# xuanvinh1997/llm-fp8

Hardware: AMD Instinct MI355X
Metric: train tokens/sec + FP8 GEMM % of MFMA peak, Llama-3.2-3B seq512 b16 (higher is better)
Workload: dtype fp8 (E4M3/E5M2 operands, fp32 accumulate, bf16 activations); 1 GPU; llama-3.2-3b (28 layers) full fine-tuning step, batch 16/GPU x seq 512, fp8_scenario=default (te_llama counterpart, lm_head FP8 under the outer recipe), random-init weights, synthetic tokens; route=fused, global_batch=16, seq_len=512, parallelism=single

## Files before the change

### include/mi_fp8.h

```cpp
#ifndef MI_FP8_H
#define MI_FP8_H

#include <stdint.h>

#ifdef __cplusplus
extern "C" {
#endif

#define MI_FMT_E4M3 0
#define MI_FMT_E5M2 1

#define MI_OK 0
#define MI_ERR_ARG (-1)
#define MI_ERR_SHAPE (-2)
#define MI_ERR_HIP (-3)

#define MI_OUT_BF16 0
#define MI_OUT_F32 1

#define MI_AMAX_ALGO_MAX 0
#define MI_AMAX_ALGO_MOST_RECENT 1

#define MI_ABI_VERSION 5
#define MI_ABI_REVISION 4
// ... 124 lines not shown
                        const float* grad_scale, float lr, float beta1, float beta2, float eps, float weight_decay,
                        int64_t step, void* stream);
int mi_adamw_cast_bf16_multi(const int64_t* table, int n_tensors, const int32_t* chunks, int n_chunks, int chunk_elems,
                             const float* grad_scale, float lr, float beta1, float beta2, float eps, float weight_decay,
                             int64_t step, void* stream);
int mi_adamw_mxcast_bf16_multi(const int64_t* table, int n_tensors, const int32_t* chunks, int n_chunks, int chunk_elems,
                               const float* grad_scale, float lr, float beta1, float beta2, float eps, float weight_decay,
                               int64_t step, void* stream);

int mi_adamw_f32_multi(const int64_t* table, int n_tensors, const int32_t* chunks, int n_chunks, int chunk_elems,
                       const float* grad_scale, float lr, float beta1, float beta2, float eps, float weight_decay,
                       int64_t step, int sink_kind, void* stream);

int mi_adamw_sr_bf16_multi(const int64_t* table, int n_tensors, const int32_t* chunks, int n_chunks, int chunk_elems,
                           const float* grad_scale, float lr, float beta1, float beta2, float eps, float weight_decay,
                           int64_t step, int sink_kind, uint64_t seed, void* stream);

int mi_embedding_grad_add(void* grad_bf16, const void* dy_bf16, const int64_t* sorted_ids, const int64_t* perm, int64_t tokens,
                          int64_t hidden, int64_t vocab, float alpha, int64_t padding_idx, void* stream);
int mi_adamw_bf16(void* p_bf16, const void* g_bf16, void* exp_avg_bf16, void* exp_avg_sq_bf16, int64_t n,
                  const float* grad_scale, float lr, float beta1, float beta2, float eps, float weight_decay,
                  int64_t step, void* stream);

int mi_attn_fwd(const void* q, const void* k, const void* v, void* o, float* lse, int B, int S, int H, int G, int D,
                int64_t q_ts, int64_t k_ts, int64_t v_ts, int64_t o_ts, float scale, int causal, void* stream);
typedef struct mi_gemm_plan {
  int algo, family, build, sched, mx, tile_cfg, tiles_m, tiles_n, grid_x, grid_y, block, one_tile_per_wg, sk_units, bias_use;
} mi_gemm_plan;
#ifdef MI_DIAG
int mi_attn_fwd_diag(const void* q, const void* k, const void* v, void* o, float* lse, unsigned long long* dbg, int B, int S,
                     int H, int G, int D, int64_t q_ts, int64_t k_ts, int64_t v_ts, int64_t o_ts, float scale, void* stream);
int mi_gemm_plan_diag(int entry, int64_t M, int64_t N, int64_t K, int64_t lda, int64_t ldb, int64_t ldd, int fmt_a, int fmt_b,
                      int out_dtype, int has_bias, int algo, mi_gemm_plan* out);
#endif
int mi_attn_bwd(const void* q, const void* k, const void* v, const void* o, const void* dout, const float* lse,
                float* delta, void* dq, void* dk, void* dv, int B, int S, int H, int G, int D, int64_t q_ts,
                int64_t k_ts, int64_t v_ts, int64_t o_ts, int64_t do_ts, int64_t dq_ts, int64_t dk_ts, int64_t dv_ts,
                float scale, int causal, void* stream);

#ifdef __cplusplus
}
#endif
#endif
```

### llm_fp8_amd/_lib.py

```python
from __future__ import annotations

import ctypes
import os

_HERE = os.path.dirname(os.path.abspath(__file__))
LIB_PATH = os.environ.get("LLM_FP8_AMD_LIB") or os.path.join(_HERE, "libmi_fp8.so")
LAB_LIB_PATH = os.path.join(os.path.dirname(_HERE), "tools", "bin", "libmi_fp8_lab.so")

MI_FMT_E4M3 = 0
MI_FMT_E5M2 = 1
ABI_VERSION = 5
ABI_REVISION = 4

_c_i64 = ctypes.c_int64
_c_int = ctypes.c_int
_p = ctypes.c_void_p

class GemmProblem(ctypes.Structure):
    _fields_ = [("A", ctypes.c_void_p), ("B", ctypes.c_void_p), ("D", ctypes.c_void_p), ("sa_inv", ctypes.c_void_p),
                ("sb_inv", ctypes.c_void_p), ("M", ctypes.c_int64), ("N", ctypes.c_int64), ("K", ctypes.c_int64),
                ("lda", ctypes.c_int64), ("ldb", ctypes.c_int64), ("ldd", ctypes.c_int64)]


class GemmMxProblem(ctypes.Structure):
# ... 48 lines not shown
    "mi_gemm_set_workspace": [_p, _c_i64],
    "mi_attn_fwd": [_p, _p, _p, _p, _p, _c_int, _c_int, _c_int, _c_int, _c_int, _c_i64, _c_i64, _c_i64, _c_i64, ctypes.c_float,
                    _c_int, _p],
    "mi_attn_bwd": [_p] * 10 + [_c_int] * 5 + [_c_i64] * 8 + [ctypes.c_float, _c_int, _p],
    "mi_mxfp8_norm_quantize": [_p, _p, _p, _p, _p, _p, _p, _c_i64, _c_i64, _c_int, _p],
    "mi_mxfp8_swiglu_quantize": [_p, _p, _p, _p, _p, _c_i64, _c_i64, _c_int, _p],
    "mi_mxfp8_dswiglu_quantize": [_p, _p, _p, _p, _p, _p, _p, _c_i64, _c_i64, _c_int, _p],
    "mi_gemm_mxfp8": [_p, _p, _p, _p, _p, _p, _c_i64, _c_i64, _c_i64, _c_int, _c_int, _c_int, _c_int, _p],
    "mi_swiglu_cast_bias": [_p, _p, _p, _p, _p, _p, _c_i64, _c_i64, _c_int, _p],
    "mi_dswiglu_cast_bias": [_p, _p, _p, _p, _p, _p, _p, _p, _c_i64, _c_i64, _c_int, _p],
    "mi_add_bias_rmsnorm_stats": [_p, _p, _p, _p, _p, _c_i64, _c_i64, ctypes.c_float, _p],
    "mi_gemm_fp8_clock": [_p, _p, _p, _p, _p, _c_i64, _c_i64, _c_i64, _c_i64, _c_i64, _c_i64, _c_int, _p, _p],
}
REVISION_SIGNATURES = {
    "mi_abi_revision": [],
    "mi_adamw_f32_multi": [_p, _c_int, _p, _c_int, _c_int, _p, ctypes.c_float, ctypes.c_float, ctypes.c_float, ctypes.c_float,
                           ctypes.c_float, _c_i64, _c_int, _p],
    "mi_amax_bf16": [_p, _p, _c_int, _c_i64, _c_i64, _p],
    "mi_amax_norm": [_p, _p, _p, _p, _c_int, _c_i64, _c_i64, _p],
    "mi_amax_swiglu": [_p, _p, _p, _c_int, _c_i64, _c_i64, _p],
    "mi_amax_dswiglu": [_p, _p, _p, _p, _c_int, _c_i64, _c_i64, _p],
    "mi_current_scale": [_p, _c_int, ctypes.c_float, ctypes.c_float, _c_int, _p, _p],
    "mi_blockfp8_quantize_ex": [_p, _p, _p, _p, _p, _p, _c_i64, _c_i64, _c_i64, _c_int, _c_int, ctypes.c_float, _p],
    "mi_blockfp8_norm_quantize": [_p, _p, _p, _p, _p, _p, _p, _c_i64, _c_i64, _c_int, _c_int, ctypes.c_float, _p],
    "mi_blockfp8_swiglu_quantize": [_p, _p, _p, _p, _p, _c_i64, _c_i64, _c_int, _c_int, ctypes.c_float, _p],
    "mi_blockfp8_dswiglu_quantize": [_p, _p, _p, _p, _p, _p, _p, _c_i64, _c_i64, _c_int, _c_int, ctypes.c_float, _p],
    "mi_adamw_sr_bf16_multi": [_p, _c_int, _p, _c_int, _c_int, _p, ctypes.c_float, ctypes.c_float, ctypes.c_float, ctypes.c_float,
                               ctypes.c_float, _c_i64, _c_int, ctypes.c_uint64, _p],
}
SIGNATURES.update(REVISION_SIGNATURES)
LAB_SIGNATURES = {
    "mi_attn_fwd_diag": [_p, _p, _p, _p, _p, _p, _c_int, _c_int, _c_int, _c_int, _c_int, _c_i64, _c_i64, _c_i64, _c_i64, ctypes.c_float, _p],
    "mi_gemm_plan_diag": [_c_int] + [_c_i64] * 6 + [_c_int] * 5 + [ctypes.POINTER(GemmPlan)],
}

_lib = None


def _bind(path: str, signatures) -> ctypes.CDLL:
    lib = ctypes.CDLL(path)
    for name, argtypes in signatures.items():
        if name in REVISION_SIGNATURES and not hasattr(lib, name):
            continue
        fn = getattr(lib, name)
        fn.argtypes = argtypes
        fn.restype = ctypes.c_char_p if name == "mi_last_error" else (_c_i64 if name == "mi_gemm_workspace_bytes" else _c_int)
    v = lib.mi_abi_version()
    if v != ABI_VERSION:
        raise ImportError(f"{os.path.basename(path)} ABI version {v} != expected {ABI_VERSION}; rebuild it")
    return lib


def load() -> ctypes.CDLL:
    global _lib
    if _lib is not None:
        return _lib
    if not os.path.exists(LIB_PATH):
        raise ImportError(
            f"{LIB_PATH} not found: the HIP extension is not built. Run "
            "`python -c 'import __graft_entry__ as g; g.build()'` or `make -C llm_fp8_amd/csrc`. "
            "llm_fp8_amd has no CPU/PyTorch fallback for the FP8 path.")
    _lib = _bind(LIB_PATH, SIGNATURES)
    return _lib


def use_lab_library() -> ctypes.CDLL:
# ... 31 lines not shown
```

### llm_fp8_amd/csrc/mi_api.hip

```cpp
#include "mi_common.h"
#include <string.h>

namespace mi {

static thread_local char g_err[512] = "";

void set_error(const char* fmt, ...) {
  va_list ap;
  va_start(ap, fmt);
  vsnprintf(g_err, sizeof(g_err), fmt, ap);
  va_end(ap);
}

int hip_fail(hipError_t e, const char* what) {
  set_error("%s: HIP error %d (%s)", what, (int)e, hipGetErrorString(e));
  return MI_ERR_HIP;
}

}

extern "C" int mi_abi_version(void) { return MI_ABI_VERSION; }
extern "C" int mi_abi_revision(void) { return MI_ABI_REVISION; }

extern "C" const char* mi_last_error(void) { return mi::g_err; }

extern "C" int mi_device_supported(void) {
  int dev = 0;
  hipError_t e = hipGetDevice(&dev);
  if (e != hipSuccess) return mi::hip_fail(e, "hipGetDevice");
  hipDeviceProp_t prop;
  e = hipGetDeviceProperties(&prop, dev);
  if (e != hipSuccess) return mi::hip_fail(e, "hipGetDeviceProperties");
  return strncmp(prop.gcnArchName, "gfx950", 6) == 0 ? 1 : 0;
}
```

### llm_fp8_amd/csrc/mi_common.h

```cpp
#pragma once
#include <hip/hip_runtime.h>
#include <float.h>
#include <stdint.h>
#include <stdio.h>
#include <stdarg.h>
#include "../../include/mi_fp8.h"

namespace mi {

void set_error(const char* fmt, ...);
int hip_fail(hipError_t e, const char* what);

#define MI_CHECK_AS(rc, cond, ...)         \
  do {                                     \
    if (!(cond)) {                         \
      mi::set_error(__VA_ARGS__);          \
      return rc;                           \
    }                                      \
  } while (0)
#define MI_CHECK_ARG(cond, ...) MI_CHECK_AS(MI_ERR_ARG, cond, __VA_ARGS__)
#define MI_CHECK_SHAPE(cond, ...) MI_CHECK_AS(MI_ERR_SHAPE, cond, __VA_ARGS__)

#define MI_CHECK_LAUNCH(what)                                   \
  do {                                                          \
// ... 25 lines not shown

template <int FMT>
__device__ __forceinline__ u32 cvt_pk_fp8(float a, float b) {
  const float mx = fp8_max_of<FMT>();
  a = __builtin_amdgcn_fmed3f(a, -mx, mx);
  b = __builtin_amdgcn_fmed3f(b, -mx, mx);
  if (FMT == MI_FMT_E4M3) return (u32)__builtin_amdgcn_cvt_pk_fp8_f32(a, b, 0, false) & 0xFFFFu;
  return (u32)__builtin_amdgcn_cvt_pk_bf8_f32(a, b, 0, false) & 0xFFFFu;
}

template <int FMT>
__device__ __forceinline__ u32 cvt4_fp8(float v0, float v1, float v2, float v3) {
  const float mx = fp8_max_of<FMT>();
  float c0 = __builtin_amdgcn_fmed3f(v0, -mx, mx), c1 = __builtin_amdgcn_fmed3f(v1, -mx, mx);
  float c2 = __builtin_amdgcn_fmed3f(v2, -mx, mx), c3 = __builtin_amdgcn_fmed3f(v3, -mx, mx);
  int r = 0;
  if (FMT == MI_FMT_E4M3) {
    r = __builtin_amdgcn_cvt_pk_fp8_f32(c0, c1, r, false);
    r = __builtin_amdgcn_cvt_pk_fp8_f32(c2, c3, r, true);
  } else {
    r = __builtin_amdgcn_cvt_pk_bf8_f32(c0, c1, r, false);
    r = __builtin_amdgcn_cvt_pk_bf8_f32(c2, c3, r, true);
  }
  u32 u = (u32)r;
  if (__builtin_expect((v0 != v0) | (v1 != v1) | (v2 != v2) | (v3 != v3), 0)) {
    if (v0 != v0) u = (u & 0xFFFFFF00u) | 0x0000007Fu;
    if (v1 != v1) u = (u & 0xFFFF00FFu) | 0x00007F00u;
    if (v2 != v2) u = (u & 0xFF00FFFFu) | 0x007F0000u;
    if (v3 != v3) u = (u & 0x00FFFFFFu) | 0x7F000000u;
  }
  return u;
}

typedef unsigned short u16x2 __attribute__((ext_vector_type(2)));
__device__ __forceinline__ u32 nan_screen(u32 acc, u32 w) {
  u16x2 a = __builtin_bit_cast(u16x2, acc), b = __builtin_bit_cast(u16x2, w & 0x7FFF7FFFu);
  return __builtin_bit_cast(u32, __builtin_elementwise_max(a, b));
}
__device__ __forceinline__ bool nan_seen(u32 acc) { return max(acc & 0xFFFFu, acc >> 16) > 0x7F80u; }

__device__ __forceinline__ u32 bperm(u32 hi, u32 lo, u32 sel) { return __builtin_amdgcn_perm(hi, lo, sel); }

__device__ __forceinline__ void transpose4x4(u32 r0, u32 r1, u32 r2, u32 r3, u32& c0, u32& c1, u32& c2,
                                             u32& c3) {
  u32 t01l = bperm(r1, r0, 0x05010400u);
  u32 t01h = bperm(r1, r0, 0x07030602u);
  u32 t23l = bperm(r3, r2, 0x05010400u);
  u32 t23h = bperm(r3, r2, 0x07030602u);
  c0 = bperm(t23l, t01l, 0x05040100u);
  c1 = bperm(t23l, t01l, 0x07060302u);
  c2 = bperm(t23h, t01h, 0x05040100u);
  c3 = bperm(t23h, t01h, 0x07060302u);
}

__device__ __forceinline__ u32 e8m0_roundup(float val) {
  u32 u = __float_as_uint(val);
  u32 e = (u >> 23) & 0xFFu, man = u & 0x7FFFFFu;
  if (man > 0 && e != 0xFEu && !(e == 0 && man <= 0x400000u)) ++e;
  if (val != val) e = 0xFFu;
  else if (isinf(val)) e = 0xFEu;
  else if (val == 0.0f) e = 0u;
  return e;
}
__device__ __forceinline__ float e8m0_inv(u32 e) {
  if (e == 0xFFu) return __uint_as_float(0x7FC00000u);
  if (e == 0xFEu) return __uint_as_float(0x00400000u);
  return __uint_as_float((254u - e) << 23);
}

__device__ __forceinline__ float scale_from_amax(float amax, float fp8_max, float eps, bool pow2) {
  const float a = amax < eps ? eps : amax;
  float scale = 1.0f;
  if (!(a == 0.0f) && !isinf(a)) {
    scale = fp8_max / a;
    if (isinf(scale)) scale = FLT_MAX;
    if (scale != scale) scale = 1.0f;
  }
  if (pow2) scale = __uint_as_float(__float_as_uint(scale) & 0xFF800000u);
  return scale;
}

__device__ __forceinline__ float wave_max(float v) {
#pragma unroll
  for (int o = 32; o >= 1; o >>= 1) v = fmaxf(v, __shfl_xor(v, o));
  return v;
}

__device__ __forceinline__ float sigmoidf_(float g) { return 1.0f / (1.0f + __expf(-g)); }

__device__ __forceinline__ void norm_value2(u32 w, float rs, float g0, float g1, float& v0, float& v1) {
  v0 = (__uint_as_float(w << 16) * rs) * g0;
  v1 = (__uint_as_float(w & 0xFFFF0000u) * rs) * g1;
}

template <int MODE>
__device__ __forceinline__ void swiglu_value2(u32 wg, u32 wu, u32 wd, bool has_bias, const float* bg, const float* bu, float* v0,
                                              float* v1) {
  float g2[2] = {__uint_as_float(wg << 16), __uint_as_float(wg & 0xFFFF0000u)};
  float u2[2] = {__uint_as_float(wu << 16), __uint_as_float(wu & 0xFFFF0000u)};
  const float d2[2] = {__uint_as_float(wd << 16), __uint_as_float(wd & 0xFFFF0000u)};
  if (has_bias) {
    g2[0] += bg[0];
    g2[1] += bg[1];
    u2[0] += bu[0];
    u2[1] += bu[1];
  }
#pragma unroll
  for (int e = 0; e < 2; ++e) {
    const float sg = sigmoidf_(g2[e]);
    if (MODE == 0) {
      v0[e] = g2[e] * sg * u2[e];
    } else {
      v0[e] = d2[e] * u2[e] * (sg * (1.0f + g2[e] * (1.0f - sg)));
      v1[e] = d2[e] * (g2[e] * sg);
    }
  }
}

}
#ifndef MI_NT_Y
#define MI_NT_Y 0
#endif
#ifndef MI_NT_YT
#define MI_NT_YT 0
#endif
#if defined(__HIPCC__)
namespace mi {
template <bool NT>
__device__ __forceinline__ void st8(uint8_t* p, unsigned int a, unsigned int b) {
  typedef unsigned int v2u_st8 __attribute__((ext_vector_type(2)));
  const v2u_st8 w = {a, b};
  if (NT) __builtin_nontemporal_store(w, reinterpret_cast<v2u_st8*>(p));
  else *reinterpret_cast<v2u_st8*>(p) = w;
}

template <bool NT>
__device__ __forceinline__ void store_rows8(uint8_t* dst, int64_t ld, const u32 (&lo)[8], const u32 (&hi)[8]) {
#pragma unroll
  for (int i = 0; i < 8; ++i) st8<NT>(dst + i * ld, lo[i], hi[i]);
}
template <bool NT>
__device__ __forceinline__ void store_cols8(uint8_t* dst, int64_t ld, const u32 (&lo)[8], const u32 (&hi)[8]) {
// ... 106 lines not shown
```

### llm_fp8_amd/csrc/mi_fused.hip

```cpp
#include "mi_common.h"

namespace mi {

template <int DIR>
__global__ __launch_bounds__(256) void rope_qkv_kernel(uint16_t* __restrict__ fused, uint16_t* __restrict__ q,
                                                       uint16_t* __restrict__ k, uint16_t* __restrict__ v,
                                                       const float* __restrict__ cosT, const float* __restrict__ sinT,
                                                       int rows, int seq, int nq, int nk, int D) {
  const int half = D >> 1;
  const int vph = half >> 3;
  const int W = (nq + 2 * nk) * D;
  const int rot_items = (nq + nk) * vph;
  const int cpy_items = (nk * D) >> 3;
  const int per_row = rot_items + cpy_items;
  const int64_t items = (int64_t)rows * per_row;
  const float sgn = DIR == 0 ? 1.0f : -1.0f;
  for (int64_t it = (int64_t)blockIdx.x * blockDim.x + threadIdx.x; it < items; it += (int64_t)gridDim.x * blockDim.x) {
    const int64_t r = it / per_row;
    const int w = (int)(it - r * per_row);
    uint16_t* frow = fused + r * W;
    if (w < rot_items) {
      const int hd = w / vph, vv = w - hd * vph;
      uint16_t* sep = hd < nq ? q + (r * nq + hd) * D : k + (r * nk + (hd - nq)) * D;
      uint16_t* f1 = frow + hd * D + vv * 8;
// ... 8 lines not shown
      *reinterpret_cast<v4f*>(c) = *reinterpret_cast<const v4f*>(cp);
      *reinterpret_cast<v4f*>(c + 4) = *reinterpret_cast<const v4f*>(cp + 4);
      *reinterpret_cast<v4f*>(sn) = *reinterpret_cast<const v4f*>(sp);
      *reinterpret_cast<v4f*>(sn + 4) = *reinterpret_cast<const v4f*>(sp + 4);
      v4i o1, o2;
#pragma unroll
      for (int j = 0; j < 4; ++j) {
        const u32 wa = (u32)a[j], wb = (u32)b[j];
        const float x1l = __uint_as_float(wa << 16), x1h = __uint_as_float(wa & 0xFFFF0000u);
        const float x2l = __uint_as_float(wb << 16), x2h = __uint_as_float(wb & 0xFFFF0000u);
        const float cl = c[2 * j], ch = c[2 * j + 1], sl = sgn * sn[2 * j], sh = sgn * sn[2 * j + 1];
        o1[j] = (int)pack_bf16x2(x1l * cl - x2l * sl, x1h * ch - x2h * sh);
        o2[j] = (int)pack_bf16x2(x2l * cl + x1l * sl, x2h * ch + x1h * sh);
      }
      *reinterpret_cast<v4i*>(out1) = o1;
      *reinterpret_cast<v4i*>(out1 + half) = o2;
    } else {
      const int cv = w - rot_items;
      uint16_t* fp = frow + (nq + nk) * D + cv * 8;
      uint16_t* sp2 = v + r * (int64_t)(nk * D) + cv * 8;
      if (DIR == 0) *reinterpret_cast<v4i*>(sp2) = *reinterpret_cast<const v4i*>(fp);
      else *reinterpret_cast<v4i*>(fp) = *reinterpret_cast<const v4i*>(sp2);
    }
  }
}

template <int FMT, bool WRITE_Y, bool WRITE_T>
__global__ __launch_bounds__(256) void rope_bwd_cast_kernel(const uint16_t* __restrict__ dq, const uint16_t* __restrict__ dk,
                                                            const uint16_t* __restrict__ dv, const float* __restrict__ cosT,
                                                            const float* __restrict__ sinT, uint8_t* __restrict__ y,
                                                            uint8_t* __restrict__ yT, const float* __restrict__ scale_p,
                                                            float* amax_out, int rows, int seq, int nq, int nk) {
  constexpr int D = 128, half = 64;
  __shared__ float s_amax[4];
  const int tid = threadIdx.x, lane = tid & 63, wave = tid >> 6;
  const int W = (nq + 2 * nk) * D;
  const int units = (nq + nk) + 2 * nk;
  const int64_t u_all = (int64_t)blockIdx.x * 4 + wave;
  const int rb = (int)(u_all / units), u = (int)(u_all % units);
  const int r0 = rb * 64 + (lane >> 3) * 8, lc = (lane & 7) * 8;
  const float scale = *scale_p;
  float amax = 0.0f;
  auto emit = [&](const float (&f)[8][8], int c0) {
    u32 lo[8], hi[8];
#pragma unroll
    for (int i = 0; i < 8; ++i) {
#pragma unroll
      for (int j = 0; j < 8; ++j) amax = fmaxf(amax, (f[i][j] != f[i][j]) ? 0.0f : fabsf(f[i][j]));
      lo[i] = cvt4_fp8<FMT>(f[i][0] * scale, f[i][1] * scale, f[i][2] * scale, f[i][3] * scale);
      hi[i] = cvt4_fp8<FMT>(f[i][4] * scale, f[i][5] * scale, f[i][6] * scale, f[i][7] * scale);
    }
    if (WRITE_Y) {
      uint8_t* dst = y + (int64_t)r0 * W + c0;
#pragma unroll
      for (int i = 0; i < 8; ++i) mi::st8<MI_NT_Y>(dst + (int64_t)i * W, lo[i], hi[i]);
    }
    if (WRITE_T) {
      u32 a[4], b[4], c[4], d[4];
      transpose4x4(lo[0], lo[1], lo[2], lo[3], a[0], a[1], a[2], a[3]);
      transpose4x4(lo[4], lo[5], lo[6], lo[7], b[0], b[1], b[2], b[3]);
      transpose4x4(hi[0], hi[1], hi[2], hi[3], c[0], c[1], c[2], c[3]);
      transpose4x4(hi[4], hi[5], hi[6], hi[7], d[0], d[1], d[2], d[3]);
      uint8_t* dst = yT + (int64_t)c0 * rows + r0;
#pragma unroll
      for (int j = 0; j < 4; ++j) {
        mi::st8<MI_NT_YT>(dst + (int64_t)j * rows, a[j], b[j]);
        mi::st8<MI_NT_YT>(dst + (int64_t)(j + 4) * rows, c[j], d[j]);
      }
    }
  };
  auto bf16_round = [](float v) { return __uint_as_float(float_to_bf16_bits(v) << 16); };
  if (r0 < rows) {
    if (u < nq + nk) {
      const int hd = u;
      const uint16_t* src = hd < nq ? dq + ((int64_t)r0 * nq + hd) * D : dk + ((int64_t)r0 * nk + (hd - nq)) * D;
      const int64_t rstride = (int64_t)(hd < nq ? nq : nk) * D;
      float f1[8][8], f2[8][8];
#pragma unroll
      for (int i = 0; i < 8; ++i) {
        const v4i a = *reinterpret_cast<const v4i*>(src + i * rstride + lc);
        const v4i b = *reinterpret_cast<const v4i*>(src + i * rstride + half + lc);
        const int pos = (r0 + i) % seq;
        float c[8], sn[8];
        *reinterpret_cast<v4f*>(c) = *reinterpret_cast<const v4f*>(cosT + (int64_t)pos * half + lc);
        *reinterpret_cast<v4f*>(c + 4) = *reinterpret_cast<const v4f*>(cosT + (int64_t)pos * half + lc + 4);
        *reinterpret_cast<v4f*>(sn) = *reinterpret_cast<const v4f*>(sinT + (int64_t)pos * half + lc);
        *reinterpret_cast<v4f*>(sn + 4) = *reinterpret_cast<const v4f*>(sinT + (int64_t)pos * half + lc + 4);
#pragma unroll
        for (int j = 0; j < 4; ++j) {
          const u32 wa = (u32)a[j], wb = (u32)b[j];
          const float x1l = __uint_as_float(wa << 16), x1h = __uint_as_float(wa & 0xFFFF0000u);
          const float x2l = __uint_as_float(wb << 16), x2h = __uint_as_float(wb & 0xFFFF0000u);
          const float cl = c[2 * j], ch = c[2 * j + 1], sl = -1.0f * sn[2 * j], sh = -1.0f * sn[2 * j + 1];
          f1[i][2 * j] = bf16_round(x1l * cl - x2l * sl);
          f1[i][2 * j + 1] = bf16_round(x1h * ch - x2h * sh);
          f2[i][2 * j] = bf16_round(x2l * cl + x1l * sl);
          f2[i][2 * j + 1] = bf16_round(x2h * ch + x1h * sh);
        }
      }
      emit(f1, hd * D + lc);
      emit(f2, hd * D + half + lc);
    } else {
      const int tc = u - (nq + nk);
      float f[8][8];
#pragma unroll
      for (int i = 0; i < 8; ++i) {
        const v4i a = *reinterpret_cast<const v4i*>(dv + (int64_t)(r0 + i) * (nk * D) + tc * 64 + lc);
#pragma unroll
        for (int j = 0; j < 4; ++j) {
          f[i][2 * j] = __uint_as_float((u32)a[j] << 16);
          f[i][2 * j + 1] = __uint_as_float((u32)a[j] & 0xFFFF0000u);
        }
      }
      emit(f, (nq + nk) * D + tc * 64 + lc);
    }
  }
  if (amax_out != nullptr) {
    amax = wave_max(amax);
    if (lane == 0) s_amax[wave] = amax;
    __syncthreads();
    if (tid == 0) {
      const float m = fmaxf(fmaxf(s_amax[0], s_amax[1]), fmaxf(s_amax[2], s_amax[3]));
      if (m > 0.0f && m > __builtin_nontemporal_load(amax_out)) atomicMax(reinterpret_cast<unsigned int*>(amax_out), __float_as_uint(m));
    }
  }
}

template <int FMT, int MODE, bool WRITE_Y, bool WRITE_T>
__global__ __launch_bounds__(256) void swiglu_cast_kernel(const uint16_t* __restrict__ h, const uint16_t* __restrict__ d,
                                                          uint8_t* __restrict__ y, uint8_t* __restrict__ yT,
                                                          const float* __restrict__ scale_p, float* amax_out,
                                                          float* __restrict__ colsum, int rows, int F, int tiles_c,
                                                          const uint16_t* __restrict__ bias) {
  __shared__ float s_col[MODE == 1 ? 2 : 1][2][128];
  constexpr int NOUT = MODE == 0 ? 1 : 2;
  const int ocols = MODE == 0 ? F : 2 * F;
  const int tid = threadIdx.x, lane = tid & 63, wave = tid >> 6;
  const int tile_r = blockIdx.x / tiles_c, tile_c = blockIdx.x % tiles_c;
  const int r0 = tile_r * 128 + (wave >> 1) * 64 + (lane >> 3) * 8;
  const int cg = tile_c * 128 + (wave & 1) * 64 + (lane & 7) * 8;
  const float scale = *scale_p;
  float amax = 0.0f;
  float csum[NOUT][8];
#pragma unroll
  for (int o = 0; o < NOUT; ++o)
#pragma unroll
    for (int j = 0; j < 8; ++j) csum[o][j] = 0.0f;
// ... 3 lines not shown
    float bg[8] = {0.f, 0.f, 0.f, 0.f, 0.f, 0.f, 0.f, 0.f}, bu[8] = {0.f, 0.f, 0.f, 0.f, 0.f, 0.f, 0.f, 0.f};
    if (bias != nullptr) {
      const v4i vg = *reinterpret_cast<const v4i*>(bias + cg), vu = *reinterpret_cast<const v4i*>(bias + F + cg);
#pragma unroll
      for (int j = 0; j < 4; ++j) {
        bg[2 * j] = __uint_as_float((u32)vg[j] << 16);
        bg[2 * j + 1] = __uint_as_float((u32)vg[j] & 0xFFFF0000u);
        bu[2 * j] = __uint_as_float((u32)vu[j] << 16);
        bu[2 * j + 1] = __uint_as_float((u32)vu[j] & 0xFFFF0000u);
      }
    }
#pragma unroll
    for (int pass = 0; pass < 2; ++pass) {
      v4i gv[4], uv[4], dv[4];
#pragma unroll
      for (int i = 0; i < 4; ++i) {
        const int64_t r = r0 + 4 * pass + i;
        gv[i] = __builtin_nontemporal_load(reinterpret_cast<const v4i*>(h + r * 2 * F + cg));
        uv[i] = __builtin_nontemporal_load(reinterpret_cast<const v4i*>(h + r * 2 * F + F + cg));
        dv[i] = MODE == 1 ? __builtin_nontemporal_load(reinterpret_cast<const v4i*>(d + r * F + cg)) : (v4i){0, 0, 0, 0};
      }
#pragma unroll
      for (int i = 0; i < 4; ++i) {
        float f[NOUT][8];
#pragma unroll
        for (int j = 0; j < 4; ++j) {
          const u32 wg = (u32)gv[i][j], wu = (u32)uv[i][j], wd = (u32)dv[i][j];
          swiglu_value2<MODE>(wg, wu, wd, bias != nullptr, bg + 2 * j, bu + 2 * j, f[0] + 2 * j, f[NOUT - 1] + 2 * j);
        }
#pragma unroll
        for (int o = 0; o < NOUT; ++o) {
#pragma unroll
          for (int j = 0; j < 8; ++j) {
            amax = fmaxf(amax, (f[o][j] != f[o][j]) ? 0.0f : fabsf(f[o][j]));
            if (MODE == 1) csum[o][j] += f[o][j];
          }
          lo[o][4 * pass + i] = cvt4_fp8<FMT>(f[o][0] * scale, f[o][1] * scale, f[o][2] * scale, f[o][3] * scale);
          hi[o][4 * pass + i] = cvt4_fp8<FMT>(f[o][4] * scale, f[o][5] * scale, f[o][6] * scale, f[o][7] * scale);
        }
      }
      if (MODE == 1) __builtin_amdgcn_sched_barrier(0);
    }
#pragma unroll
    for (int o = 0; o < NOUT; ++o) {
      const int c0 = cg + o * F;
      if (WRITE_Y) store_rows8<MI_NT_Y>(y + (int64_t)r0 * ocols + c0, ocols, lo[o], hi[o]);
      if (WRITE_T) store_cols8<MI_NT_YT>(yT + (int64_t)c0 * rows + r0, rows, lo[o], hi[o]);
    }
  }
  if (MODE == 1 && colsum != nullptr) {
#pragma unroll
    for (int o = 0; o < NOUT; ++o)
#pragma unroll
      for (int j = 0; j < 8; ++j) {
        float v = csum[o][j];
        v += __shfl_xor(v, 8);
        v += __shfl_xor(v, 16);
        v += __shfl_xor(v, 32);
        if ((lane >> 3) == 0) s_col[o][wave >> 1][(wave & 1) * 64 + (lane & 7) * 8 + j] = v;
      }
    __syncthreads();
    const int c = tile_c * 128 + (tid & 127), o = tid >> 7;
    if (c < F) colsum[(int64_t)tile_r * ocols + o * F + c] = s_col[MODE == 1 ? o : 0][0][tid & 127] + s_col[MODE == 1 ? o : 0][1][tid & 127];
  }
  publish_amax(amax, amax_out);
}

template <int MODE>
static int launch_swiglu(int fmt, const void* h, const void* d, void* y, void* yT, const float* scale, float* amax, float* colsum,
                         int64_t rows, int64_t F, void* stream, const void* bias = nullptr) {
  const int tiles_r = (int)((rows + 127) / 128), tiles_c = (int)((F + 127) / 128);
// ... 264 lines not shown
}

template <int FMT, bool WRITE_Y, bool WRITE_T>
__global__ __launch_bounds__(256) void ce_bwd_cast_kernel(const uint16_t* __restrict__ x, const int64_t* __restrict__ labels,
                                                          const float* __restrict__ lse, const float* __restrict__ gscale,
                                                          uint8_t* __restrict__ y, uint8_t* __restrict__ yT,
                                                          const float* __restrict__ scale_p, float* amax_out, int rows, int cols,
                                                          int tiles_c) {
  const int tid = threadIdx.x, lane = tid & 63, wave = tid >> 6;
  const int tile_r = blockIdx.x / tiles_c, tile_c = blockIdx.x % tiles_c;
  const int r0 = tile_r * 128 + (wave >> 1) * 64 + (lane >> 3) * 8;
  const int c0 =tile_c * 128 + (wave & 1) * 64 + (lane & 7) * 8;
  const float scale = *scale_p, g0 = *gscale;
  float amax = 0.0f;
  if ((r0 < rows) && (c0 < cols)) {
    u32 lo[8], hi[8];
#pragma unroll
    for (int i = 0; i < 8; ++i) {
      const int64_t lab = labels[r0 + i];
      const bool valid = lab >= 0 && lab < cols;
      const float gs = valid ? g0 : 0.0f;
      const float l = lse[r0 + i];
      const v4i raw = __builtin_nontemporal_load(reinterpret_cast<const v4i*>(x + (int64_t)(r0 + i) * cols + c0));
      float f[8];
#pragma unroll
      for (int j = 0; j < 4; ++j) {
        float p0 = __expf(__uint_as_float((u32)raw[j] << 16) - l), p1 = __expf(__uint_as_float((u32)raw[j] & 0xFFFF0000u) - l);
        if (c0 + 2 * j == lab) p0 -= 1.0f;
        if (c0 + 2 * j + 1 == lab) p1 -= 1.0f;
        f[2 * j] = __uint_as_float(float_to_bf16_bits(p0 * gs) << 16);
        f[2 * j + 1] = __uint_as_float(float_to_bf16_bits(p1 * gs) << 16);
      }
#pragma unroll
      for (int j = 0; j < 8; ++j) amax = fmaxf(amax, (f[j] != f[j]) ? 0.0f : fabsf(f[j]));
      lo[i] = cvt4_fp8<FMT>(f[0] * scale, f[1] * scale, f[2] * scale, f[3] * scale);
      hi[i] = cvt4_fp8<FMT>(f[4] * scale, f[5] * scale, f[6] * scale, f[7] * scale);
    }
    if (WRITE_Y) store_rows8<MI_NT_Y>(y + (int64_t)r0 * cols + c0, cols, lo, hi);
    if (WRITE_T) store_cols8<MI_NT_YT>(yT + (int64_t)c0 * rows + r0, rows, lo, hi);
  }
  publish_amax(amax, amax_out);
}

}

extern "C" int mi_rope_qkv(void* fused_bf16, void* q_bf16, void* k_bf16, void* v_bf16, const float* cos_tab,
                           const float* sin_tab, int64_t rows, int64_t seq, int n_q_heads, int n_kv_heads, int head_dim,
                           int backward, void* stream) {
  MI_CHECK_ARG(fused_bf16 && q_bf16 && k_bf16 && v_bf16 && cos_tab && sin_tab, "mi_rope_qkv: null pointer");
  MI_CHECK_ARG(rows >= 0 && seq > 0 && n_q_heads > 0 && n_kv_heads > 0, "mi_rope_qkv: bad shape");
  MI_CHECK_ARG(head_dim > 0 && head_dim % 16 == 0, "mi_rope_qkv: head_dim must be a multiple of 16");
  MI_CHECK_ARG(((uintptr_t)fused_bf16 % 16) == 0 && ((uintptr_t)q_bf16 % 16) == 0 && ((uintptr_t)k_bf16 % 16) == 0 &&
                   ((uintptr_t)v_bf16 % 16) == 0 && ((uintptr_t)cos_tab % 16) == 0 && ((uintptr_t)sin_tab % 16) == 0,
               "mi_rope_qkv: pointers must be 16-byte aligned");
  MI_CHECK_ARG(rows < (1LL << 31), "mi_rope_qkv: too many rows");
  if (rows == 0) return MI_OK;
  const int64_t per_row = (int64_t)(n_q_heads + n_kv_heads) * (head_dim / 16) + (int64_t)n_kv_heads * head_dim / 8;
  int64_t blocks = (rows * per_row + 255) / 256;
  if (blocks > 8192) blocks = 8192;
  if (backward)
    hipLaunchKernelGGL(mi::rope_qkv_kernel<1>, dim3((unsigned)blocks), dim3(256), 0, (hipStream_t)stream, (uint16_t*)fused_bf16,
                       (uint16_t*)q_bf16, (uint16_t*)k_bf16, (uint16_t*)v_bf16, cos_tab, sin_tab, (int)rows, (int)seq, n_q_heads,
                       n_kv_heads, head_dim);
  else
    hipLaunchKernelGGL(mi::rope_qkv_kernel<0>, dim3((unsigned)blocks), dim3(256), 0, (hipStream_t)stream, (uint16_t*)fused_bf16,
                       (uint16_t*)q_bf16, (uint16_t*)k_bf16, (uint16_t*)v_bf16, cos_tab, sin_tab, (int)rows, (int)seq, n_q_heads,
                       n_kv_heads, head_dim);
  MI_CHECK_LAUNCH("mi_rope_qkv launch");
  return MI_OK;
// ... 241 lines not shown
```

Measured before the change: 87950 tokens/s.

## Speed up fused FP8 cast epilogues with fast sigmoid, NaN-deferred conversion, rope pipelining

Replaces the IEEE division in sigmoid with a hardware reciprocal plus Newton refinement, falling back to division when a wave sees large denominators. Adds a packed 8-value FP8 conversion that clamps with med3 and patches NaNs only on a rare slow path, and drops per-element NaN checks from the amax reductions. Restructures the rope/QKV backward cast kernel to load rows in pairs, carry packed outputs instead of float tiles, and recompute with NaN patching only if a NaN was seen. A diagnostic entry point is added to check fast sigmoid against IEEE bit-for-bit. These changes target ALU cost and register pressure in memory-bound elementwise kernels, with some risk around NaN and amax semantics.

```diff
diff --git a/include/mi_fp8.h b/include/mi_fp8.h
--- a/include/mi_fp8.h
+++ b/include/mi_fp8.h
@@ -180,6 +180,7 @@
                      int H, int G, int D, int64_t q_ts, int64_t k_ts, int64_t v_ts, int64_t o_ts, float scale, void* stream);
 int mi_gemm_plan_diag(int entry, int64_t M, int64_t N, int64_t K, int64_t lda, int64_t ldb, int64_t ldd, int fmt_a, int fmt_b,
                       int out_dtype, int has_bias, int algo, mi_gemm_plan* out);
+int mi_sigmoid_diag(unsigned int first_bits, unsigned long long count, unsigned long long* out, void* stream);
 #endif
 int mi_attn_bwd(const void* q, const void* k, const void* v, const void* o, const void* dout, const float* lse,
                 float* delta, void* dq, void* dk, void* dv, int B, int S, int H, int G, int D, int64_t q_ts,
diff --git a/llm_fp8_amd/_lib.py b/llm_fp8_amd/_lib.py
--- a/llm_fp8_amd/_lib.py
+++ b/llm_fp8_amd/_lib.py
@@ -104,6 +104,7 @@
 LAB_SIGNATURES = {
     "mi_attn_fwd_diag": [_p, _p, _p, _p, _p, _p, _c_int, _c_int, _c_int, _c_int, _c_int, _c_i64, _c_i64, _c_i64, _c_i64, ctypes.c_float, _p],
     "mi_gemm_plan_diag": [_c_int] + [_c_i64] * 6 + [_c_int] * 5 + [ctypes.POINTER(GemmPlan)],
+    "mi_sigmoid_diag": [ctypes.c_uint32, ctypes.c_uint64, ctypes.POINTER(ctypes.c_uint64), _p],
 }
 
 _lib = None
diff --git a/llm_fp8_amd/csrc/mi_api.hip b/llm_fp8_amd/csrc/mi_api.hip
--- a/llm_fp8_amd/csrc/mi_api.hip
+++ b/llm_fp8_amd/csrc/mi_api.hip
@@ -24,6 +24,54 @@
 
 extern "C" const char* mi_last_error(void) { return mi::g_err; }
 
+#ifdef MI_DIAG
+namespace mi {
+__global__ __launch_bounds__(256) void sigmoid_diag_kernel(u32 first, unsigned long long count, unsigned long long* out) {
+  const unsigned long long stride = (unsigned long long)gridDim.x * 256u;
+  for (unsigned long long base = (unsigned long long)blockIdx.x * 256u; base < count; base += stride) {
+    const unsigned long long i = base + threadIdx.x;
+    const float g = __uint_as_float(first + (u32)i);
+    const u32 fast = __float_as_uint(sigmoidf_(g)), ieee = __float_as_uint(sigmoid_ieee_(g));
+    if (i < count && fast != ieee) {
+      atomicAdd(out, 1ull);
+      atomicMin(out + 1, i);
+    }
+  }
+}
+__global__ void sigmoid_diag_first_kernel(u32 first, unsigned long long* out) {
+  if (out[0] == 0) return;
+  const u32 bits = first + (u32)out[1];
+  const float g = __uint_as_float(bits);
+  out[1] = bits;
+  out[2] = __float_as_uint(rcp_fast_(sigmoid_den_(g)));
+  out[3] = __float_as_uint(sigmoid_ieee_(g));
+}
+}
+
+extern "C" int mi_sigmoid_diag(unsigned int first_bits, unsigned long long count, unsigned long long* out, void* stream) {
+  MI_CHECK_ARG(out != nullptr, "mi_sigmoid_diag: null out");
+  MI_CHECK_ARG(count >= 1 && count <= (1ull << 32), "mi_sigmoid_diag: count must be in 1 .. 2^32");
+  unsigned long long* dev = nullptr;
+  hipError_t e = hipMalloc(&dev, 4 * sizeof(unsigned long long));
+  if (e != hipSuccess) return mi::hip_fail(e, "mi_sigmoid_diag: hipMalloc");
+  const unsigned long long init[4] = {0ull, ~0ull, 0ull, 0ull};
+  hipStream_t st = (hipStream_t)stream;
+  e = hipMemcpyAsync(dev, init, sizeof(init), hipMemcpyHostToDevice, st);
+  if (e == hipSuccess) {
+    const unsigned long long blocks = (count + 255) / 256;
+    hipLaunchKernelGGL(mi::sigmoid_diag_kernel, dim3((unsigned)(blocks < 16384 ? blocks : 16384)), dim3(256), 0, st, first_bits, count, dev);
+    hipLaunchKernelGGL(mi::sigmoid_diag_first_kernel, dim3(1), dim3(1), 0, st, first_bits, dev);
+    e = hipGetLastError();
+  }
+  if (e == hipSuccess) e = hipMemcpyAsync(out, dev, 4 * sizeof(unsigned long long), hipMemcpyDeviceToHost, st);
+  if (e == hipSuccess) e = hipStreamSynchronize(st);
+  (void)hipFree(dev);
+  if (e != hipSuccess) return mi::hip_fail(e, "mi_sigmoid_diag");
+  if (out[0] == 0) out[1] = 0;
+  return MI_OK;
+}
+#endif
+
 extern "C" int mi_device_supported(void) {
   int dev = 0;
   hipError_t e = hipGetDevice(&dev);
diff --git a/llm_fp8_amd/csrc/mi_common.h b/llm_fp8_amd/csrc/mi_common.h
--- a/llm_fp8_amd/csrc/mi_common.h
+++ b/llm_fp8_amd/csrc/mi_common.h
@@ -81,6 +81,45 @@
   return u;
 }
 
+template <int FMT>
+__device__ __forceinline__ bool cvt8_fp8_raw(const float (&v)[8], float scale, u32& lo, u32& hi) {
+  const float mx = fp8_max_of<FMT>();
+  float s[8], c[8];
+#pragma unroll
+  for (int j = 0; j < 8; ++j) {
+    s[j] = v[j] * scale;
+    c[j] = __builtin_amdgcn_fmed3f(s[j], -mx, mx);
+  }
+  int r0 = 0, r1 = 0;
+  if (FMT == MI_FMT_E4M3) {
+    r0 = __builtin_amdgcn_cvt_pk_fp8_f32(c[0], c[1], r0, false);
+    r0 = __builtin_amdgcn_cvt_pk_fp8_f32(c[2], c[3], r0, true);
+    r1 = __builtin_amdgcn_cvt_pk_fp8_f32(c[4], c[5], r1, false);
+    r1 = __builtin_amdgcn_cvt_pk_fp8_f32(c[6], c[7], r1, true);
+  } else {
+    r0 = __builtin_amdgcn_cvt_pk_bf8_f32(c[0], c[1], r0, false);
+    r0 = __builtin_amdgcn_cvt_pk_bf8_f32(c[2], c[3], r0, true);
+    r1 = __builtin_amdgcn_cvt_pk_bf8_f32(c[4], c[5], r1, false);
+    r1 = __builtin_amdgcn_cvt_pk_bf8_f32(c[6], c[7], r1, true);
+  }
+  lo = (u32)r0;
+  hi = (u32)r1;
+  return __builtin_isunordered(s[0], s[1]) | __builtin_isunordered(s[2], s[3]) | __builtin_isunordered(s[4], s[5]) |
+         __builtin_isunordered(s[6], s[7]);
+}
+__device__ __forceinline__ void cvt8_fp8_patch(const float (&v)[8], float scale, u32& lo, u32& hi) {
+#pragma unroll
+  for (int j = 0; j < 4; ++j) {
+    const float s0 = v[j] * scale, s1 = v[j + 4] * scale;
+    if (s0 != s0) lo = (lo & ~(0xFFu << (8 * j))) | (0x7Fu << (8 * j));
+    if (s1 != s1) hi = (hi & ~(0xFFu << (8 * j))) | (0x7Fu << (8 * j));
+  }
+}
+template <int FMT>
+__device__ __forceinline__ void cvt8_fp8(const float (&v)[8], float scale, u32& lo, u32& hi) {
+  if (__builtin_expect(cvt8_fp8_raw<FMT>(v, scale, lo, hi), 0)) cvt8_fp8_patch(v, scale, lo, hi);
+}
+
 typedef unsigned short u16x2 __attribute__((ext_vector_type(2)));
 __device__ __forceinline__ u32 nan_screen(u32 acc, u32 w) {
   u16x2 a = __builtin_bit_cast(u16x2, acc), b = __builtin_bit_cast(u16x2, w & 0x7FFF7FFFu);
@@ -135,7 +174,31 @@
   return v;
 }
 
-__device__ __forceinline__ float sigmoidf_(float g) { return 1.0f / (1.0f + __expf(-g)); }
+__device__ __forceinline__ float sigmoid_den_(float g) { return 1.0f + __expf(-g); }
+__device__ __forceinline__ float sigmoid_ieee_(float g) { return 1.0f / sigmoid_den_(g); }
+__device__ __forceinline__ bool rcp_fast_ok_(float den) { return __float_as_uint(den) < 0x7E800000u; }
+__device__ __forceinline__ float rcp_fast_(float den) {
+  const float r = __builtin_amdgcn_rcpf(den);
+  const float r1 = __builtin_fmaf(__builtin_fmaf(-den, r, 1.0f), r, r);
+  const float q = 1.0f * r1;
+  const float q1 = __builtin_fmaf(__builtin_fmaf(-den, q, 1.0f), r1, q);
+  return __builtin_fmaf(__builtin_fmaf(-den, q1, 1.0f), r1, q1);
+}
+__device__ __forceinline__ void sigmoid2_(float g0, float g1, float& s0, float& s1) {
+  const float d0 = sigmoid_den_(g0), d1 = sigmoid_den_(g1);
+  if (__builtin_expect(__builtin_amdgcn_ballot_w64(!(rcp_fast_ok_(d0) && rcp_fast_ok_(d1))) == 0, 1)) {
+    s0 = rcp_fast_(d0);
+    s1 = rcp_fast_(d1);
+  } else {
+    s0 = 1.0f / d0;
+    s1 = 1.0f / d1;
+  }
+}
+__device__ __forceinline__ float sigmoidf_(float g) {
+  const float den = sigmoid_den_(g);
+  if (__builtin_expect(__builtin_amdgcn_ballot_w64(!rcp_fast_ok_(den)) == 0, 1)) return rcp_fast_(den);
+  return 1.0f / den;
+}
 
 __device__ __forceinline__ void norm_value2(u32 w, float rs, float g0, float g1, float& v0, float& v1) {
   v0 = (__uint_as_float(w << 16) * rs) * g0;
@@ -154,9 +217,11 @@
     u2[0] += bu[0];
     u2[1] += bu[1];
   }
+  float sg2[2];
+  sigmoid2_(g2[0], g2[1], sg2[0], sg2[1]);
 #pragma unroll
   for (int e = 0; e < 2; ++e) {
-    const float sg = sigmoidf_(g2[e]);
+    const float sg = sg2[e];
     if (MODE == 0) {
       v0[e] = g2[e] * sg * u2[e];
     } else {
diff --git a/llm_fp8_amd/csrc/mi_fused.hip b/llm_fp8_amd/csrc/mi_fused.hip
--- a/llm_fp8_amd/csrc/mi_fused.hip
+++ b/llm_fp8_amd/csrc/mi_fused.hip
@@ -64,6 +64,7 @@
                                                             uint8_t* __restrict__ yT, const float* __restrict__ scale_p,
                                                             float* amax_out, int rows, int seq, int nq, int nk) {
   constexpr int D = 128, half = 64;
+  constexpr int RP = 2;
   __shared__ float s_amax[4];
   const int tid = threadIdx.x, lane = tid & 63, wave = tid >> 6;
   const int W = (nq + 2 * nk) * D;
@@ -73,15 +74,7 @@
   const int r0 = rb * 64 + (lane >> 3) * 8, lc = (lane & 7) * 8;
   const float scale = *scale_p;
   float amax = 0.0f;
-  auto emit = [&](const float (&f)[8][8], int c0) {
-    u32 lo[8], hi[8];
-#pragma unroll
-    for (int i = 0; i < 8; ++i) {
-#pragma unroll
-      for (int j = 0; j < 8; ++j) amax = fmaxf(amax, (f[i][j] != f[i][j]) ? 0.0f : fabsf(f[i][j]));
-      lo[i] = cvt4_fp8<FMT>(f[i][0] * scale, f[i][1] * scale, f[i][2] * scale, f[i][3] * scale);
-      hi[i] = cvt4_fp8<FMT>(f[i][4] * scale, f[i][5] * scale, f[i][6] * scale, f[i][7] * scale);
-    }
+  auto store = [&](const u32 (&lo)[8], const u32 (&hi)[8], int c0) {
     if (WRITE_Y) {
       uint8_t* dst = y + (int64_t)r0 * W + c0;
 #pragma unroll
@@ -103,48 +96,113 @@
   };
   auto bf16_round = [](float v) { return __uint_as_float(float_to_bf16_bits(v) << 16); };
   if (r0 < rows) {
-    if (u < nq + nk) {
-      const int hd = u;
-      const uint16_t* src = hd < nq ? dq + ((int64_t)r0 * nq + hd) * D : dk + ((int64_t)r0 * nk + (hd - nq)) * D;
-      const int64_t rstride = (int64_t)(hd < nq ? nq : nk) * D;
-      float f1[8][8], f2[8][8];
+    const bool rot = u < nq + nk;
+    const int hd = u, tc = u - (nq + nk);
+    u32 lo1[8], hi1[8], lo2[8], hi2[8];
+    const uint16_t* src = hd < nq ? dq + ((int64_t)r0 * nq + hd) * D : dk + ((int64_t)r0 * nk + (hd - nq)) * D;
+    const int64_t rstride = (int64_t)(hd < nq ? nq : nk) * D;
+    const uint16_t* vsrc = dv + (int64_t)r0 * (nk * D) + tc * 64 + lc;
+    auto rot_row = [&](const v4i& a, const v4i& b, const v4f (&c)[2], const v4f (&sn)[2], bool patch, u32 (&w)[4]) -> bool {
+      float f1[8], f2[8];
+#pragma unroll
+      for (int j = 0; j < 4; ++j) {
+        const u32 wa = (u32)a[j], wb = (u32)b[j];
+        const float x1l = __uint_as_float(wa << 16), x1h = __uint_as_float(wa & 0xFFFF0000u);
+        const float x2l = __uint_as_float(wb << 16), x2h = __uint_as_float(wb & 0xFFFF0000u);
+        const float cl = c[j >> 1][2 * (j & 1)], ch = c[j >> 1][2 * (j & 1) + 1];
+        const float sl = -1.0f * sn[j >> 1][2 * (j & 1)], sh = -1.0f * sn[j >> 1][2 * (j & 1) + 1];
+        f1[2 * j] = bf16_round(x1l * cl - x2l * sl);
+        f1[2 * j + 1] = bf16_round(x1h * ch - x2h * sh);
+        f2[2 * j] = bf16_round(x2l * cl + x1l * sl);
+        f2[2 * j + 1] = bf16_round(x2h * ch + x1h * sh);
+      }
+#pragma unroll
+      for (int j = 0; j < 8; ++j) amax = fmaxf(amax, fmaxf(fabsf(f1[j]), fabsf(f2[j])));
+      const bool n1 = cvt8_fp8_raw<FMT>(f1, scale, w[0], w[1]), n2 = cvt8_fp8_raw<FMT>(f2, scale, w[2], w[3]);
+      if (patch) {
+        cvt8_fp8_patch(f1, scale, w[0], w[1]);
+        cvt8_fp8_patch(f2, scale, w[2], w[3]);
+      }
+      return n1 | n2;
+    };
+    auto v_row = [&](const v4i& a, bool patch, u32 (&w)[4]) -> bool {
+      float f[8];
+#pragma unroll
+      for (int j = 0; j < 4; ++j) {
+        f[2 * j] = __uint_as_float((u32)a[j] << 16);
+        f[2 * j + 1] = __uint_as_float((u32)a[j] & 0xFFFF0000u);
+      }
+#pragma unroll
+      for (int j = 0; j < 8; ++j) amax = fmaxf(amax, (f[j] != f[j]) ? 0.0f : fabsf(f[j]));
+      const bool n = cvt8_fp8_raw<FMT>(f, scale, w[0], w[1]);
+      if (patch) cvt8_fp8_patch(f, scale, w[0], w[1]);
+      return n;
+    };
+    const int pos0 = r0 % seq;
+    auto next_pos = [&](int pos) { return pos + 1 == seq ? 0 : pos + 1; };
+    auto load_cs = [&](int pos, v4f (&c)[2], v4f (&sn)[2]) {
+      c[0] = *reinterpret_cast<const v4f*>(cosT + (int64_t)pos * half + lc);
+      c[1] = *reinterpret_cast<const v4f*>(cosT + (int64_t)pos * half + lc + 4);
+      sn[0] = *reinterpret_cast<const v4f*>(sinT + (int64_t)pos * half + lc);
+      sn[1] = *reinterpret_cast<const v4f*>(sinT + (int64_t)pos * half + lc + 4);
+    };
+    bool nan = false;
+    if (rot) {
+      int pos = pos0;
+#pragma unroll
+      for (int pass = 0; pass < 8 / RP; ++pass) {
+        v4i av[RP], bv[RP];
+        v4f cv[RP][2], sv[RP][2];
+#pragma unroll
+        for (int i = 0; i < RP; ++i) {
+          av[i] = *reinterpret_cast<const v4i*>(src + (RP * pass + i) * rstride + lc);
+          bv[i] = *reinterpret_cast<const v4i*>(src + (RP * pass + i) * rstride + half + lc);
+          load_cs(pos, cv[i], sv[i]);
+          pos = next_pos(pos);
+        }
+#pragma unroll
+        for (int i = 0; i < RP; ++i) {
+          u32 w[4];
+          nan |= rot_row(av[i], bv[i], cv[i], sv[i], false, w);
+          lo1[RP * pass + i] = w[0], hi1[RP * pass + i] = w[1], lo2[RP * pass + i] = w[2], hi2[RP * pass + i] = w[3];
+        }
+        __builtin_amdgcn_sched_barrier(0);
+      }
+    } else {
+      v4i av[8];
+#pragma unroll
+      for (int i = 0; i < 8; ++i) av[i] = *reinterpret_cast<const v4i*>(vsrc + (int64_t)i * (nk * D));
 #pragma unroll
       for (int i = 0; i < 8; ++i) {
-        const v4i a = *reinterpret_cast<const v4i*>(src + i * rstride + lc);
-        const v4i b = *reinterpret_cast<const v4i*>(src + i * rstride + half + lc);
-        const int pos = (r0 + i) % seq;
-        float c[8], sn[8];
-        *reinterpret_cast<v4f*>(c) = *reinterpret_cast<const v4f*>(cosT + (int64_t)pos * half + lc);
-        *reinterpret_cast<v4f*>(c + 4) = *reinterpret_cast<const v4f*>(cosT + (int64_t)pos * half + lc + 4);
-        *reinterpret_cast<v4f*>(sn) = *reinterpret_cast<const v4f*>(sinT + (int64_t)pos * half + lc);
-        *reinterpret_cast<v4f*>(sn + 4) = *reinterpret_cast<const v4f*>(sinT + (int64_t)pos * half + lc + 4);
-#pragma unroll
-        for (int j = 0; j < 4; ++j) {
-          const u32 wa = (u32)a[j], wb = (u32)b[j];
-          const float x1l = __uint_as_float(wa << 16), x1h = __uint_as_float(wa & 0xFFFF0000u);
-          const float x2l = __uint_as_float(wb << 16), x2h = __uint_as_float(wb & 0xFFFF0000u);
-          const float cl = c[2 * j], ch = c[2 * j + 1], sl = -1.0f * sn[2 * j], sh = -1.0f * sn[2 * j + 1];
-          f1[i][2 * j] = bf16_round(x1l * cl - x2l * sl);
-          f1[i][2 * j + 1] = bf16_round(x1h * ch - x2h * sh);
-          f2[i][2 * j] = bf16_round(x2l * cl + x1l * sl);
-          f2[i][2 * j + 1] = bf16_round(x2h * ch + x1h * sh);
+        u32 w[4];
+        nan |= v_row(av[i], false, w);
+        lo1[i] = w[0], hi1[i] = w[1];
+      }
+    }
+    if (__builtin_expect(nan, 0)) {
+      int pos = pos0;
+#pragma unroll
+      for (int r = 0; r < 8; ++r) {
+        u32 w[4];
+        if (rot) {
+          v4f c[2], sn[2];
+          load_cs(pos, c, sn);
+          pos = next_pos(pos);
+          rot_row(*reinterpret_cast<const v4i*>(src + r * rstride + lc), *reinterpret_cast<const v4i*>(src + r * rstride + half + lc), c,
+                  sn, true, w);
+          lo2[r] = w[2], hi2[r] = w[3];
+        } else {
+          v_row(*reinterpret_cast<const v4i*>(vsrc + (int64_t)r * (nk * D)), true, w);
         }
-      }
-      emit(f1, hd * D + lc);
-      emit(f2, hd * D + half + lc);
+        lo1[r] = w[0], hi1[r] = w[1];
+        __builtin_amdgcn_sched_barrier(0);
+      }
+    }
+    if (rot) {
+      store(lo1, hi1, hd * D + lc);
+      store(lo2, hi2, hd * D + half + lc);
     } else {
-      const int tc = u - (nq + nk);
-      float f[8][8];
-#pragma unroll
-      for (int i = 0; i < 8; ++i) {
-        const v4i a = *reinterpret_cast<const v4i*>(dv + (int64_t)(r0 + i) * (nk * D) + tc * 64 + lc);
-#pragma unroll
-        for (int j = 0; j < 4; ++j) {
-          f[i][2 * j] = __uint_as_float((u32)a[j] << 16);
-          f[i][2 * j + 1] = __uint_as_float((u32)a[j] & 0xFFFF0000u);
-        }
-      }
-      emit(f, (nq + nk) * D + tc * 64 + lc);
+      store(lo1, hi1, (nq + nk) * D + tc * 64 + lc);
     }
   }
   if (amax_out != nullptr) {
@@ -214,11 +272,10 @@
         for (int o = 0; o < NOUT; ++o) {
 #pragma unroll
           for (int j = 0; j < 8; ++j) {
-            amax = fmaxf(amax, (f[o][j] != f[o][j]) ? 0.0f : fabsf(f[o][j]));
+            amax = fmaxf(amax, fabsf(f[o][j]));
             if (MODE == 1) csum[o][j] += f[o][j];
           }
-          lo[o][4 * pass + i] = cvt4_fp8<FMT>(f[o][0] * scale, f[o][1] * scale, f[o][2] * scale, f[o][3] * scale);
-          hi[o][4 * pass + i] = cvt4_fp8<FMT>(f[o][4] * scale, f[o][5] * scale, f[o][6] * scale, f[o][7] * scale);
+          cvt8_fp8<FMT>(f[o], scale, lo[o][4 * pass + i], hi[o][4 * pass + i]);
         }
       }
       if (MODE == 1) __builtin_amdgcn_sched_barrier(0);
@@ -549,9 +606,8 @@
         f[2 * j + 1] = __uint_as_float(float_to_bf16_bits(p1 * gs) << 16);
       }
 #pragma unroll
-      for (int j = 0; j < 8; ++j) amax = fmaxf(amax, (f[j] != f[j]) ? 0.0f : fabsf(f[j]));
-      lo[i] = cvt4_fp8<FMT>(f[0] * scale, f[1] * scale, f[2] * scale, f[3] * scale);
-      hi[i] = cvt4_fp8<FMT>(f[4] * scale, f[5] * scale, f[6] * scale, f[7] * scale);
+      for (int j = 0; j < 8; ++j) amax = fmaxf(amax, fabsf(f[j]));
+      cvt8_fp8<FMT>(f, scale, lo[i], hi[i]);
     }
     if (WRITE_Y) store_rows8<MI_NT_Y>(y + (int64_t)r0 * cols + c0, cols, lo, hi);
     if (WRITE_T) store_cols8<MI_NT_YT>(yT + (int64_t)c0 * rows + r0, rows, lo, hi);
```

After: 89630 tokens/s (median of 6 runs). No clear change (+1.9%).
